# BSVogler/k8s-runpod-kubelet

Hardware: AMD Instinct MI355X
Metric: gpu_pods_scheduled_per_sec (higher is better)
Workload: dtype n/a; 1 GPU; podworker HIP init+kernel per pod (gfx950); model=gpu-pod-lifecycle, global_batch=1, seq_len=0, parallelism=1 kubelet x 1 GPUs, 8 sync workers, lifecycle=create->bind->launch->Ready->delete->finalized, burst_size=0, pods_total=10

## Files before the change

### k8s_runpod_kubelet_amd/ops/build.py

```python

from __future__ import annotations

import os
import shlex
import subprocess
import sys
import sysconfig
from pathlib import Path

OPS_DIR = Path(__file__).resolve().parent
CSRC = OPS_DIR / "csrc"
PODWORKER_DIR = OPS_DIR / "podworker"
GPUCHECK_DIR = OPS_DIR / "gpucheck"

GFX_ARCH = os.environ.get("PYTORCH_ROCM_ARCH", "gfx950")
HIPCC = os.environ.get("HIPCC", "/opt/rocm/bin/hipcc")
CXX = os.environ.get("CXX", "g++")


def _run(cmd: list[str]) -> None:
    print("+", " ".join(shlex.quote(c) for c in cmd), flush=True)
    subprocess.run(cmd, check=True)


def ext_suffix() -> str:
    return sysconfig.get_config_var("EXT_SUFFIX") or ".so"


def native_ext_path() -> Path:
    return OPS_DIR / f"_native{ext_suffix()}"


def podworker_path() -> Path:
    return PODWORKER_DIR / "podworker"


def gpucheck_path() -> Path:
    return GPUCHECK_DIR / "gpucheck"


def _content_stamp(sources: list[Path], cmd: list[str]) -> str:
    import hashlib

    h = hashlib.sha256()
    for s in sources:
        h.update(s.name.encode())
        h.update(s.read_bytes())
    h.update("\0".join(cmd).encode())
    return h.hexdigest()


def _is_fresh(target: Path, stamp_file: Path, stamp: str) -> bool:
    if not target.exists():
        return False
    try:
        return stamp_file.read_text().strip() == stamp
    except OSError:
        return False


def build_native(force: bool = False) -> Path:
    import pybind11

    out = native_ext_path()
    sources = [CSRC / "module.cpp", CSRC / "probe.cpp", CSRC / "launcher.cpp"]
    headers = [CSRC / "probe.h", CSRC / "launcher.h"]
    cmd = [
        CXX, "-O2", "-g", "-std=c++17", "-shared", "-fPIC",
        "-fvisibility=hidden",
        f"-I{pybind11.get_include()}",
        f"-I{sysconfig.get_paths()['include']}",
        *[str(s) for s in sources],
        "-o", str(out),
    ]
    stamp_file = OPS_DIR / ".native.buildstamp"
    stamp = _content_stamp(sources + headers, cmd)
    if not force and _is_fresh(out, stamp_file, stamp):
        return out
    _run(cmd)
    stamp_file.write_text(stamp + "\n")
    return out


def build_podworker(force: bool = False) -> Path:
    out = podworker_path()
    src = PODWORKER_DIR / "podworker.hip"
    cmd = [
        HIPCC, f"--offload-arch={GFX_ARCH}", "-O2", "-std=c++17",
        str(src), "-o", str(out),
    ]
    stamp_file = PODWORKER_DIR / ".podworker.buildstamp"
    stamp = _content_stamp([src], cmd)
    if not force and _is_fresh(out, stamp_file, stamp):
        return out
    _run(cmd)
    stamp_file.write_text(stamp + "\n")
    return out


def build_gpucheck(force: bool = False) -> Path:
    out = gpucheck_path()
    src = GPUCHECK_DIR / "gpucheck.hip"
    header = GPUCHECK_DIR / "gpucheck_pattern.h"
    cmd = [
        HIPCC, f"--offload-arch={GFX_ARCH}", "-O2", "-std=c++17",
        str(src), "-o", str(out),
    ]
    stamp_file = GPUCHECK_DIR / ".gpucheck.buildstamp"
    stamp = _content_stamp([src, header], cmd)
    if not force and _is_fresh(out, stamp_file, stamp):
        return out
    _run(cmd)
    stamp_file.write_text(stamp + "\n")
    return out


def build_all(force: bool = False) -> None:
    build_native(force=force)
    build_podworker(force=force)
    build_gpucheck(force=force)


if __name__ == "__main__":
    build_all(force="--force" in sys.argv)
```

### k8s_runpod_kubelet_amd/ops/podworker/podworker.hip

```cpp

#include <hip/hip_runtime.h>

#include <arpa/inet.h>
#include <netinet/in.h>
#include <signal.h>
#include <stdio.h>
#include <stdlib.h>
#include <string.h>
#include <sys/socket.h>
#include <time.h>
#include <unistd.h>

#include <string>
#include <vector>

#define HIP_CHECK(expr)                                                     \
  do {                                                                      \
    hipError_t err_ = (expr);                                               \
    if (err_ != hipSuccess) {                                               \
      fprintf(stderr, "podworker: %s failed: %s\n", #expr,                  \
              hipGetErrorString(err_));                                     \
      return 11;                                                            \
    }                                                                       \
  } while (0)

__global__ void touch_kernel(unsigned int* out, int n) {
  int i = blockIdx.x * blockDim.x + threadIdx.x;
  if (i < n) out[i] = static_cast<unsigned int>(i) * 2u + 1u;
}

static volatile sig_atomic_t g_terminate = 0;
static void on_term(int) { g_terminate = 1; }

static int touch_gpus(int expect_gpus) {
  int count = 0;
  HIP_CHECK(hipGetDeviceCount(&count));
  if (expect_gpus >= 0 && count != expect_gpus) {
    fprintf(stderr, "podworker: visible GPU count %d != expected %d\n", count,
            expect_gpus);
    return 12;
  }
  const int n = 1 << 20;
  for (int dev = 0; dev < count; ++dev) {
    HIP_CHECK(hipSetDevice(dev));
    unsigned int* d = nullptr;
    HIP_CHECK(hipMalloc(&d, n * sizeof(unsigned int)));
    dim3 block(256);
    dim3 grid((n + 255) / 256);
    hipLaunchKernelGGL(touch_kernel, grid, block, 0, 0, d, n);
    HIP_CHECK(hipGetLastError());
    const int head = 1 << 16;
    std::vector<unsigned int> host(head + 1);
    HIP_CHECK(hipMemcpy(host.data(), d, head * sizeof(unsigned int),
                        hipMemcpyDeviceToHost));
    HIP_CHECK(hipMemcpy(host.data() + head, d + (n - 1),
                        sizeof(unsigned int), hipMemcpyDeviceToHost));
    HIP_CHECK(hipFree(d));
    for (int i = 0; i < head; i += 4099) {
      if (host[i] != static_cast<unsigned int>(i) * 2u + 1u) {
        fprintf(stderr, "podworker: kernel verify failed at %d on dev %d\n", i,
                dev);
        return 13;
      }
    }
    if (host[head] != static_cast<unsigned int>(n - 1) * 2u + 1u) {
      fprintf(stderr, "podworker: kernel verify failed at tail on dev %d\n",
              dev);
      return 13;
    }
    hipDeviceProp_t prop;
    HIP_CHECK(hipGetDeviceProperties(&prop, dev));
    printf("podworker: dev %d %s gcnArch=%s vram=%zuMB ok\n", dev, prop.name,
           prop.gcnArchName, prop.totalGlobalMem >> 20);
  }
  return 0;
}

static int listen_on(int port) {
  int fd = socket(AF_INET, SOCK_STREAM | SOCK_CLOEXEC, 0);
  if (fd < 0) return -1;
  int one = 1;
  setsockopt(fd, SOL_SOCKET, SO_REUSEADDR, &one, sizeof(one));
  sockaddr_in addr{};
  addr.sin_family = AF_INET;
  addr.sin_addr.s_addr = htonl(INADDR_ANY);
  addr.sin_port = htons(static_cast<uint16_t>(port));
  if (bind(fd, reinterpret_cast<sockaddr*>(&addr), sizeof(addr)) != 0 ||
      listen(fd, 8) != 0) {
    close(fd);
    return -1;
  }
  return fd;
}

int main(int argc, char** argv) {
  int expect_gpus = -1;
  double run_for = -1.0;
  bool hold = false;
  int exit_code = 0;
  double startup_delay = 0.0;
  std::vector<int> ports;

  for (int i = 1; i < argc; ++i) {
    std::string a = argv[i];
    auto next = [&]() -> const char* { return (i + 1 < argc) ? argv[++i] : ""; };
    if (a == "--expect-gpus") expect_gpus = atoi(next());
    else if (a == "--run-for") run_for = atof(next());
    else if (a == "--hold") hold = true;
    else if (a == "--exit-code") exit_code = atoi(next());
    else if (a == "--startup-delay") startup_delay = atof(next());
    else if (a == "--listen-port") ports.push_back(atoi(next()));
    else if (a == "--fail") {
      fprintf(stderr, "podworker: simulated failure\n");
      return 1;
    } else {
      fprintf(stderr, "podworker: unknown arg %s\n", a.c_str());
      return 2;
    }
  }

  struct sigaction sa{};
  sa.sa_handler = on_term;
  sigaction(SIGTERM, &sa, nullptr);
  sigaction(SIGINT, &sa, nullptr);

  if (startup_delay > 0) usleep(static_cast<useconds_t>(startup_delay * 1e6));

  if (expect_gpus >= 0) {
    int rc = touch_gpus(expect_gpus);
    if (rc != 0) return rc;
  }

  std::vector<int> listen_fds;
  for (int p : ports) {
    int fd = listen_on(p);
    if (fd < 0) {
      fprintf(stderr, "podworker: listen on %d failed\n", p);
      return 3;
    }
    listen_fds.push_back(fd);
  }

  const char* ready_env = getenv("AMDVK_READY_FD");
  if (ready_env) {
    int fd = atoi(ready_env);
    const char msg[] = "READY\n";
    ssize_t w = write(fd, msg, sizeof(msg) - 1);
    (void)w;
    close(fd);
  }
  printf("podworker: ready (gpus=%d ports=%zu)\n", expect_gpus, ports.size());
  fflush(stdout);

  if (hold && run_for < 0) {
    while (!g_terminate) pause();
  } else if (run_for > 0) {
    double remaining = run_for;
    while (remaining > 0 && !g_terminate) {
      double chunk = remaining > 0.1 ? 0.1 : remaining;
      usleep(static_cast<useconds_t>(chunk * 1e6));
      remaining -= chunk;
    }
  }
  for (int fd : listen_fds) close(fd);
  printf("podworker: exiting code=%d\n", exit_code);
  return exit_code;
}
```

Measured before the change: 3.084 pods/s.

## Replace HIP runtime in podworker with direct HSA dispatch of embedded code object

The podworker no longer links the HIP runtime. It initializes HSA directly, loads a prebuilt code object embedded in the binary, and dispatches the touch kernel and a new gather kernel through AQL packets on one queue. Verification reads only the sampled elements from fine-grained host memory instead of copying them back with memcpy. The process exits via _exit to skip runtime teardown. The intent is to cut HIP runtime initialization and shutdown from each pod's startup and exit, at the cost of a more complex build (code-object extraction, metadata parsing) and hand-written queue and packet handling.

After: 3.676 pods/s (median of 6 runs). +19.2%, better.

```diff
diff --git a/k8s_runpod_kubelet_amd/ops/build.py b/k8s_runpod_kubelet_amd/ops/build.py
--- a/k8s_runpod_kubelet_amd/ops/build.py
+++ b/k8s_runpod_kubelet_amd/ops/build.py
@@ -82,18 +82,83 @@
     return out
 
 
+def _kernarg_offsets(notes: str) -> dict[str, list[int]]:
+    import re
+
+    kernels: dict[str, list[int]] = {}
+    body = notes.split("amdhsa.kernels:", 1)[1].split("\namdhsa.", 1)[0]
+    for block in re.split(r"^  - ", body, flags=re.M)[1:]:
+        name = re.search(r"^    \.name:\s+(\S+)", block, flags=re.M)
+        if not name:
+            raise RuntimeError("kernel metadata entry without a .name")
+        args = re.search(r"^    \.args:\n((?:      .*\n)*)", block, flags=re.M)
+        offsets = []
+        for arg in re.split(r"^      - ", args.group(1) if args else "",
+                            flags=re.M)[1:]:
+            if re.search(r"\.value_kind:\s+hidden_", arg):
+                continue
+            offsets.append(int(re.search(r"\.offset:\s+(\d+)", arg).group(1)))
+        kernels[name.group(1)] = offsets
+    return kernels
+
+
+def _write_kernels_inc(code_object: Path, notes: str, inc: Path) -> None:
+    offsets = _kernarg_offsets(notes)
+    expected = {"touch_kernel": 2, "gather_kernel": 4}
+    for name, nargs in expected.items():
+        if len(offsets.get(name, [])) != nargs:
+            raise RuntimeError(
+                f"{code_object.name}: expected {nargs} explicit arguments for "
+                f"{name}, metadata gives {offsets.get(name)}")
+    data = code_object.read_bytes()
+    lines = ["// generated by ops/build.py from podworker_kernels.hip",
+             "alignas(4096) static const unsigned char kPwCodeObject[] = {"]
+    for i in range(0, len(data), 16):
+        lines.append("  " + ",".join(str(b) for b in data[i:i + 16]) + ",")
+    lines.append("};")
+    for var, name in (("kTouchArgOffsets", "touch_kernel"),
+                      ("kGatherArgOffsets", "gather_kernel")):
+        lines.append(f"static const size_t {var}[] = "
+                     f"{{{', '.join(map(str, offsets[name]))}}};")
+    inc.write_text("\n".join(lines) + "\n")
+
+
 def build_podworker(force: bool = False) -> Path:
     out = podworker_path()
-    src = PODWORKER_DIR / "podworker.hip"
-    cmd = [
+    host_src = PODWORKER_DIR / "podworker.hip"
+    dev_src = PODWORKER_DIR / "podworker_kernels.hip"
+    code_object = PODWORKER_DIR / "podworker_kernels.co"
+    inc = PODWORKER_DIR / "podworker_kernels.inc"
+    staged = PODWORKER_DIR / "podworker.new"
+    readelf = subprocess.run(
+        [HIPCC, "-print-prog-name=llvm-readelf"], check=True,
+        capture_output=True, text=True).stdout.strip()
+    rocm = Path(os.environ.get("ROCM_PATH") or Path(readelf).resolve().parents[3])
+    rocm_lib = (rocm / "lib").resolve()
+    dev_cmd = [
         HIPCC, f"--offload-arch={GFX_ARCH}", "-O2", "-std=c++17",
-        str(src), "-o", str(out),
+        "--cuda-device-only", "--no-gpu-bundle-output",
+        str(dev_src), "-o", str(code_object),
+    ]
+    notes_cmd = [readelf, "--notes", str(code_object)]
+    host_cmd = [
+        CXX, "-O2", "-std=c++17", "-x", "c++", str(host_src), "-x", "none",
+        f"-I{rocm / 'include'}", f"-L{rocm_lib}", "-lhsa-runtime64",
+        f"-Wl,--enable-new-dtags,-rpath,{rocm_lib}",
+        "-o", str(staged),
     ]
     stamp_file = PODWORKER_DIR / ".podworker.buildstamp"
-    stamp = _content_stamp([src], cmd)
+    stamp = _content_stamp([host_src, dev_src],
+                           dev_cmd + notes_cmd + host_cmd)
     if not force and _is_fresh(out, stamp_file, stamp):
         return out
-    _run(cmd)
+    _run(dev_cmd)
+    print("+", " ".join(shlex.quote(c) for c in notes_cmd), flush=True)
+    notes = subprocess.run(notes_cmd, check=True, capture_output=True,
+                           text=True).stdout
+    _write_kernels_inc(code_object, notes, inc)
+    _run(host_cmd)
+    os.replace(staged, out)
     stamp_file.write_text(stamp + "\n")
     return out
 
diff --git a/k8s_runpod_kubelet_amd/ops/podworker/podworker.hip b/k8s_runpod_kubelet_amd/ops/podworker/podworker.hip
--- a/k8s_runpod_kubelet_amd/ops/podworker/podworker.hip
+++ b/k8s_runpod_kubelet_amd/ops/podworker/podworker.hip
@@ -1,9 +1,11 @@
 
-#include <hip/hip_runtime.h>
+#include <hsa/hsa.h>
+#include <hsa/hsa_ext_amd.h>
 
 #include <arpa/inet.h>
 #include <netinet/in.h>
 #include <signal.h>
+#include <stdint.h>
 #include <stdio.h>
 #include <stdlib.h>
 #include <string.h>
@@ -14,64 +16,367 @@
 #include <string>
 #include <vector>
 
-#define HIP_CHECK(expr)                                                     \
+#include "podworker_kernels.inc"
+
+[[noreturn]] static void finish(int code) {
+  fflush(stdout);
+  fflush(stderr);
+  _exit(code);
+}
+
+static const char* status_text(hsa_status_t st) {
+  const char* s = nullptr;
+  if (hsa_status_string(st, &s) == HSA_STATUS_SUCCESS && s) return s;
+  static char buf[32];
+  snprintf(buf, sizeof(buf), "HSA status 0x%x", static_cast<unsigned>(st));
+  return buf;
+}
+
+#define HSA_CHECK(expr)                                                     \
   do {                                                                      \
-    hipError_t err_ = (expr);                                               \
-    if (err_ != hipSuccess) {                                               \
+    hsa_status_t st_ = (expr);                                              \
+    if (st_ != HSA_STATUS_SUCCESS && st_ != HSA_STATUS_INFO_BREAK) {        \
       fprintf(stderr, "podworker: %s failed: %s\n", #expr,                  \
-              hipGetErrorString(err_));                                     \
-      return 11;                                                            \
+              status_text(st_));                                            \
+      finish(11);                                                           \
     }                                                                       \
   } while (0)
 
-__global__ void touch_kernel(unsigned int* out, int n) {
-  int i = blockIdx.x * blockDim.x + threadIdx.x;
-  if (i < n) out[i] = static_cast<unsigned int>(i) * 2u + 1u;
-}
-
 static volatile sig_atomic_t g_terminate = 0;
 static void on_term(int) { g_terminate = 1; }
 
-static int touch_gpus(int expect_gpus) {
-  int count = 0;
-  HIP_CHECK(hipGetDeviceCount(&count));
+static double now_ms() {
+  timespec ts;
+  clock_gettime(CLOCK_MONOTONIC, &ts);
+  return ts.tv_sec * 1e3 + ts.tv_nsec * 1e-6;
+}
+
+struct Timing {
+  double runtime_init = 0, queue = 0, load = 0, alloc = 0, dispatch_verify = 0;
+};
+
+static volatile int g_queue_error = 0;
+static volatile hsa_status_t g_queue_status = HSA_STATUS_SUCCESS;
+static void on_queue_error(hsa_status_t st, hsa_queue_t*, void*) {
+  fprintf(stderr, "podworker: queue error: %s\n", status_text(st));
+  g_queue_status = st;
+  g_queue_error = 1;
+}
+
+struct Agents {
+  std::vector<hsa_agent_t> gpus;
+  std::vector<hsa_agent_t> cpus;
+};
+
+static hsa_status_t collect_agent(hsa_agent_t agent, void* data) {
+  hsa_device_type_t type;
+  hsa_status_t st = hsa_agent_get_info(agent, HSA_AGENT_INFO_DEVICE, &type);
+  if (st != HSA_STATUS_SUCCESS) return st;
+  auto* a = static_cast<Agents*>(data);
+  if (type == HSA_DEVICE_TYPE_GPU) a->gpus.push_back(agent);
+  else if (type == HSA_DEVICE_TYPE_CPU) a->cpus.push_back(agent);
+  return HSA_STATUS_SUCCESS;
+}
+
+struct PoolQuery {
+  bool want_kernarg, want_fine, want_coarse;
+  bool found;
+  hsa_amd_memory_pool_t pool;
+};
+
+static hsa_status_t match_pool(hsa_amd_memory_pool_t pool, void* data) {
+  auto* q = static_cast<PoolQuery*>(data);
+  hsa_amd_segment_t seg;
+  hsa_status_t st = hsa_amd_memory_pool_get_info(
+      pool, HSA_AMD_MEMORY_POOL_INFO_SEGMENT, &seg);
+  if (st != HSA_STATUS_SUCCESS) return st;
+  if (seg != HSA_AMD_SEGMENT_GLOBAL) return HSA_STATUS_SUCCESS;
+  bool can_alloc = false;
+  st = hsa_amd_memory_pool_get_info(
+      pool, HSA_AMD_MEMORY_POOL_INFO_RUNTIME_ALLOC_ALLOWED, &can_alloc);
+  if (st != HSA_STATUS_SUCCESS) return st;
+  if (!can_alloc) return HSA_STATUS_SUCCESS;
+  uint32_t flags = 0;
+  st = hsa_amd_memory_pool_get_info(
+      pool, HSA_AMD_MEMORY_POOL_INFO_GLOBAL_FLAGS, &flags);
+  if (st != HSA_STATUS_SUCCESS) return st;
+  if (q->want_kernarg && !(flags & HSA_AMD_MEMORY_POOL_GLOBAL_FLAG_KERNARG_INIT))
+    return HSA_STATUS_SUCCESS;
+  if (q->want_fine && !(flags & HSA_AMD_MEMORY_POOL_GLOBAL_FLAG_FINE_GRAINED))
+    return HSA_STATUS_SUCCESS;
+  if (q->want_coarse &&
+      !(flags & HSA_AMD_MEMORY_POOL_GLOBAL_FLAG_COARSE_GRAINED))
+    return HSA_STATUS_SUCCESS;
+  q->pool = pool;
+  q->found = true;
+  return HSA_STATUS_INFO_BREAK;
+}
+
+static bool find_pool(const std::vector<hsa_agent_t>& agents, bool kernarg,
+                      bool fine, bool coarse, hsa_amd_memory_pool_t* out) {
+  for (hsa_agent_t a : agents) {
+    PoolQuery q{kernarg, fine, coarse, false, {}};
+    HSA_CHECK(hsa_amd_agent_iterate_memory_pools(a, match_pool, &q));
+    if (q.found) {
+      *out = q.pool;
+      return true;
+    }
+  }
+  return false;
+}
+
+static hsa_status_t first_isa(hsa_isa_t isa, void* data) {
+  *static_cast<hsa_isa_t*>(data) = isa;
+  return HSA_STATUS_INFO_BREAK;
+}
+
+struct Kernel {
+  uint64_t object = 0;
+  uint32_t kernarg_size = 0, group_size = 0, private_size = 0;
+};
+
+static Kernel lookup_kernel(hsa_executable_t exec, hsa_agent_t agent,
+                            const char* name) {
+  hsa_executable_symbol_t sym;
+  HSA_CHECK(hsa_executable_get_symbol_by_name(exec, name, &agent, &sym));
+  Kernel k;
+  HSA_CHECK(hsa_executable_symbol_get_info(
+      sym, HSA_EXECUTABLE_SYMBOL_INFO_KERNEL_OBJECT, &k.object));
+  HSA_CHECK(hsa_executable_symbol_get_info(
+      sym, HSA_EXECUTABLE_SYMBOL_INFO_KERNEL_KERNARG_SEGMENT_SIZE,
+      &k.kernarg_size));
+  HSA_CHECK(hsa_executable_symbol_get_info(
+      sym, HSA_EXECUTABLE_SYMBOL_INFO_KERNEL_GROUP_SEGMENT_SIZE,
+      &k.group_size));
+  HSA_CHECK(hsa_executable_symbol_get_info(
+      sym, HSA_EXECUTABLE_SYMBOL_INFO_KERNEL_PRIVATE_SEGMENT_SIZE,
+      &k.private_size));
+  return k;
+}
+
+template <typename T>
+static void put_arg(char* kernarg, const Kernel& k, size_t offset, T value) {
+  if (offset + sizeof(T) > k.kernarg_size) {
+    fprintf(stderr, "podworker: kernarg offset %zu past segment size %u\n",
+            offset, k.kernarg_size);
+    finish(11);
+  }
+  memcpy(kernarg + offset, &value, sizeof(T));
+}
+
+static const uint32_t kBlock = 256;
+static const uint32_t kQueuePackets = 64;
+static const unsigned int kPoison = 0xDEADBEEFu;
+
+static void fill_dispatch(hsa_kernel_dispatch_packet_t* p, const Kernel& k,
+                          uint32_t items, void* kernarg,
+                          hsa_signal_t completion) {
+  p->workgroup_size_x = kBlock;
+  p->workgroup_size_y = 1;
+  p->workgroup_size_z = 1;
+  p->reserved0 = 0;
+  p->grid_size_x = (items + kBlock - 1) / kBlock * kBlock;
+  p->grid_size_y = 1;
+  p->grid_size_z = 1;
+  p->private_segment_size = k.private_size;
+  p->group_segment_size = k.group_size;
+  p->kernel_object = k.object;
+  p->kernarg_address = kernarg;
+  p->reserved2 = 0;
+  p->completion_signal = completion;
+}
+
+static void publish(hsa_kernel_dispatch_packet_t* p, bool barrier) {
+  uint16_t header =
+      (HSA_PACKET_TYPE_KERNEL_DISPATCH << HSA_PACKET_HEADER_TYPE) |
+      ((barrier ? 1 : 0) << HSA_PACKET_HEADER_BARRIER) |
+      (HSA_FENCE_SCOPE_SYSTEM << HSA_PACKET_HEADER_SCACQUIRE_FENCE_SCOPE) |
+      (HSA_FENCE_SCOPE_SYSTEM << HSA_PACKET_HEADER_SCRELEASE_FENCE_SCOPE);
+  uint16_t setup = 1 << HSA_KERNEL_DISPATCH_PACKET_SETUP_DIMENSIONS;
+  __atomic_store_n(reinterpret_cast<uint32_t*>(p),
+                   header | (static_cast<uint32_t>(setup) << 16),
+                   __ATOMIC_RELEASE);
+}
+
+static int touch_gpus(int expect_gpus, int n, bool verify_all, Timing* tm) {
+  double t0 = now_ms();
+  HSA_CHECK(hsa_init());
+  Agents agents;
+  HSA_CHECK(hsa_iterate_agents(collect_agent, &agents));
+  int count = static_cast<int>(agents.gpus.size());
   if (expect_gpus >= 0 && count != expect_gpus) {
     fprintf(stderr, "podworker: visible GPU count %d != expected %d\n", count,
             expect_gpus);
     return 12;
   }
-  const int n = 1 << 20;
+  uint64_t ticks_per_s = 0;
+  HSA_CHECK(hsa_system_get_info(HSA_SYSTEM_INFO_TIMESTAMP_FREQUENCY,
+                                &ticks_per_s));
+  hsa_amd_memory_pool_t kernarg_pool{}, host_pool{};
+  if (count > 0) {
+    if (!find_pool(agents.cpus, true, false, false, &kernarg_pool)) {
+      fprintf(stderr, "podworker: kernarg pool lookup failed: none found\n");
+      return 11;
+    }
+    if (!find_pool(agents.cpus, false, true, false, &host_pool)) {
+      fprintf(stderr,
+              "podworker: fine-grained system pool lookup failed: none found\n");
+      return 11;
+    }
+  }
+  tm->runtime_init += now_ms() - t0;
+
+  std::vector<int> sample;
+  if (verify_all) {
+    sample.resize(n);
+    for (int i = 0; i < n; ++i) sample[i] = i;
+  } else {
+    const int head = n < (1 << 16) ? n : (1 << 16);
+    for (int i = 0; i < head; i += 4099) sample.push_back(i);
+    sample.push_back(n - 1);
+  }
+  const int m = static_cast<int>(sample.size());
+
   for (int dev = 0; dev < count; ++dev) {
-    HIP_CHECK(hipSetDevice(dev));
-    unsigned int* d = nullptr;
-    HIP_CHECK(hipMalloc(&d, n * sizeof(unsigned int)));
-    dim3 block(256);
-    dim3 grid((n + 255) / 256);
-    hipLaunchKernelGGL(touch_kernel, grid, block, 0, 0, d, n);
-    HIP_CHECK(hipGetLastError());
-    const int head = 1 << 16;
-    std::vector<unsigned int> host(head + 1);
-    HIP_CHECK(hipMemcpy(host.data(), d, head * sizeof(unsigned int),
-                        hipMemcpyDeviceToHost));
-    HIP_CHECK(hipMemcpy(host.data() + head, d + (n - 1),
-                        sizeof(unsigned int), hipMemcpyDeviceToHost));
-    HIP_CHECK(hipFree(d));
-    for (int i = 0; i < head; i += 4099) {
-      if (host[i] != static_cast<unsigned int>(i) * 2u + 1u) {
-        fprintf(stderr, "podworker: kernel verify failed at %d on dev %d\n", i,
-                dev);
+    hsa_agent_t gpu = agents.gpus[dev];
+
+    t0 = now_ms();
+    hsa_amd_memory_pool_t vram_pool{};
+    if (!find_pool({gpu}, false, false, true, &vram_pool)) {
+      fprintf(stderr,
+              "podworker: device memory pool lookup failed: none on dev %d\n",
+              dev);
+      return 11;
+    }
+    tm->runtime_init += now_ms() - t0;
+
+    t0 = now_ms();
+    hsa_queue_t* queue = nullptr;
+    HSA_CHECK(hsa_queue_create(gpu, kQueuePackets, HSA_QUEUE_TYPE_SINGLE,
+                               on_queue_error, nullptr, UINT32_MAX, UINT32_MAX,
+                               &queue));
+    tm->queue += now_ms() - t0;
+
+    t0 = now_ms();
+    hsa_code_object_reader_t reader;
+    HSA_CHECK(hsa_code_object_reader_create_from_memory(
+        kPwCodeObject, sizeof(kPwCodeObject), &reader));
+    hsa_executable_t exec;
+    HSA_CHECK(hsa_executable_create_alt(
+        HSA_PROFILE_FULL, HSA_DEFAULT_FLOAT_ROUNDING_MODE_DEFAULT, nullptr,
+        &exec));
+    HSA_CHECK(hsa_executable_load_agent_code_object(exec, gpu, reader, nullptr,
+                                                    nullptr));
+    HSA_CHECK(hsa_executable_freeze(exec, nullptr));
+    Kernel touch = lookup_kernel(exec, gpu, "touch_kernel.kd");
+    Kernel gather = lookup_kernel(exec, gpu, "gather_kernel.kd");
+    tm->load += now_ms() - t0;
+
+    t0 = now_ms();
+    unsigned int* out = nullptr;
+    int* idx = nullptr;
+    unsigned int* dst = nullptr;
+    char* kernarg = nullptr;
+    HSA_CHECK(hsa_amd_memory_pool_allocate(
+        vram_pool, static_cast<size_t>(n) * sizeof(unsigned int), 0,
+        reinterpret_cast<void**>(&out)));
+    HSA_CHECK(hsa_amd_memory_pool_allocate(
+        host_pool, static_cast<size_t>(m) * sizeof(int), 0,
+        reinterpret_cast<void**>(&idx)));
+    HSA_CHECK(hsa_amd_memory_pool_allocate(
+        host_pool, static_cast<size_t>(m) * sizeof(unsigned int), 0,
+        reinterpret_cast<void**>(&dst)));
+    const size_t gather_at = (touch.kernarg_size + 63u) & ~size_t(63);
+    const size_t kernarg_bytes = gather_at + gather.kernarg_size;
+    HSA_CHECK(hsa_amd_memory_pool_allocate(
+        kernarg_pool, kernarg_bytes, 0, reinterpret_cast<void**>(&kernarg)));
+    HSA_CHECK(hsa_amd_agents_allow_access(1, &gpu, nullptr, idx));
+    HSA_CHECK(hsa_amd_agents_allow_access(1, &gpu, nullptr, dst));
+    HSA_CHECK(hsa_amd_agents_allow_access(1, &gpu, nullptr, kernarg));
+    hsa_signal_t done;
+    HSA_CHECK(hsa_signal_create(1, 0, nullptr, &done));
+    tm->alloc += now_ms() - t0;
+
+    t0 = now_ms();
+    memcpy(idx, sample.data(), static_cast<size_t>(m) * sizeof(int));
+    for (int j = 0; j < m; ++j) dst[j] = kPoison;
+    memset(kernarg, 0, kernarg_bytes);
+    put_arg(kernarg, touch, kTouchArgOffsets[0], out);
+    put_arg(kernarg, touch, kTouchArgOffsets[1], n);
+    char* gather_args = kernarg + gather_at;
+    put_arg(gather_args, gather, kGatherArgOffsets[0],
+            static_cast<const unsigned int*>(out));
+    put_arg(gather_args, gather, kGatherArgOffsets[1],
+            static_cast<const int*>(idx));
+    put_arg(gather_args, gather, kGatherArgOffsets[2], dst);
+    put_arg(gather_args, gather, kGatherArgOffsets[3], m);
+
+    const uint64_t at = hsa_queue_add_write_index_relaxed(queue, 2);
+    auto* ring = static_cast<hsa_kernel_dispatch_packet_t*>(queue->base_address);
+    const uint32_t mask = queue->size - 1;
+    hsa_kernel_dispatch_packet_t* p0 = &ring[at & mask];
+    hsa_kernel_dispatch_packet_t* p1 = &ring[(at + 1) & mask];
+    fill_dispatch(p0, touch, static_cast<uint32_t>(n), kernarg,
+                  hsa_signal_t{0});
+    fill_dispatch(p1, gather, static_cast<uint32_t>(m), gather_args, done);
+    publish(p0, false);
+    publish(p1, true);
+    hsa_signal_store_screlease(queue->doorbell_signal,
+                               static_cast<hsa_signal_value_t>(at + 1));
+
+    const uint64_t slice = ticks_per_s / 10;
+    bool completed = false;
+    for (int s = 0; s < 100 && !g_queue_error; ++s) {
+      if (hsa_signal_wait_scacquire(done, HSA_SIGNAL_CONDITION_LT, 1, slice,
+                                    HSA_WAIT_STATE_BLOCKED) < 1) {
+        completed = true;
+        break;
+      }
+    }
+    if (g_queue_error) {
+      fprintf(stderr, "podworker: kernel dispatch failed: %s\n",
+              status_text(g_queue_status));
+      return 11;
+    }
+    if (!completed) {
+      fprintf(stderr,
+              "podworker: completion signal wait failed: timed out after 10 s\n");
+      return 11;
+    }
+
+    for (int j = 0; j < m; ++j) {
+      const int i = sample[j];
+      if (dst[j] != static_cast<unsigned int>(i) * 2u + 1u) {
+        if (!verify_all && j == m - 1)
+          fprintf(stderr, "podworker: kernel verify failed at tail on dev %d\n",
+                  dev);
+        else
+          fprintf(stderr, "podworker: kernel verify failed at %d on dev %d\n",
+                  i, dev);
         return 13;
       }
     }
-    if (host[head] != static_cast<unsigned int>(n - 1) * 2u + 1u) {
-      fprintf(stderr, "podworker: kernel verify failed at tail on dev %d\n",
-              dev);
-      return 13;
-    }
-    hipDeviceProp_t prop;
-    HIP_CHECK(hipGetDeviceProperties(&prop, dev));
-    printf("podworker: dev %d %s gcnArch=%s vram=%zuMB ok\n", dev, prop.name,
-           prop.gcnArchName, prop.totalGlobalMem >> 20);
+    tm->dispatch_verify += now_ms() - t0;
+
+    char product[64] = {0};
+    HSA_CHECK(hsa_agent_get_info(
+        gpu, static_cast<hsa_agent_info_t>(HSA_AMD_AGENT_INFO_PRODUCT_NAME),
+        product));
+    hsa_isa_t isa{};
+    HSA_CHECK(hsa_agent_iterate_isas(gpu, first_isa, &isa));
+    uint32_t isa_len = 0;
+    HSA_CHECK(hsa_isa_get_info_alt(isa, HSA_ISA_INFO_NAME_LENGTH, &isa_len));
+    std::string isa_name(isa_len + 1, '\0');
+    HSA_CHECK(hsa_isa_get_info_alt(isa, HSA_ISA_INFO_NAME, &isa_name[0]));
+    isa_name.resize(strlen(isa_name.c_str()));
+    const char prefix[] = "amdgcn-amd-amdhsa--";
+    if (isa_name.compare(0, sizeof(prefix) - 1, prefix) == 0)
+      isa_name.erase(0, sizeof(prefix) - 1);
+    size_t vram_bytes = 0;
+    HSA_CHECK(hsa_amd_memory_pool_get_info(
+        vram_pool, HSA_AMD_MEMORY_POOL_INFO_SIZE, &vram_bytes));
+    printf("podworker: dev %d %s gcnArch=%s vram=%zuMB ok\n", dev, product,
+           isa_name.c_str(), vram_bytes >> 20);
   }
   return 0;
 }
@@ -94,12 +399,15 @@
 }
 
 int main(int argc, char** argv) {
+  const double t_main = now_ms();
   int expect_gpus = -1;
   double run_for = -1.0;
   bool hold = false;
   int exit_code = 0;
   double startup_delay = 0.0;
   std::vector<int> ports;
+  long long touch_elems = 1 << 20;
+  bool verify_all = false;
 
   for (int i = 1; i < argc; ++i) {
     std::string a = argv[i];
@@ -110,13 +418,24 @@
     else if (a == "--exit-code") exit_code = atoi(next());
     else if (a == "--startup-delay") startup_delay = atof(next());
     else if (a == "--listen-port") ports.push_back(atoi(next()));
+    else if (a == "--touch-elems") touch_elems = atoll(next());
+    else if (a == "--verify-all") verify_all = true;
     else if (a == "--fail") {
       fprintf(stderr, "podworker: simulated failure\n");
-      return 1;
+      finish(1);
     } else {
       fprintf(stderr, "podworker: unknown arg %s\n", a.c_str());
-      return 2;
-    }
+      finish(2);
+    }
+  }
+  if (touch_elems < 1 || touch_elems > (1ll << 28)) {
+    fprintf(stderr, "podworker: --touch-elems must be in 1..%lld\n", 1ll << 28);
+    finish(2);
+  }
+  if (verify_all && touch_elems > (1 << 20)) {
+    fprintf(stderr, "podworker: --verify-all takes at most %d elements\n",
+            1 << 20);
+    finish(2);
   }
 
   struct sigaction sa{};
@@ -126,9 +445,11 @@
 
   if (startup_delay > 0) usleep(static_cast<useconds_t>(startup_delay * 1e6));
 
+  Timing tm;
   if (expect_gpus >= 0) {
-    int rc = touch_gpus(expect_gpus);
-    if (rc != 0) return rc;
+    int rc = touch_gpus(expect_gpus, static_cast<int>(touch_elems), verify_all,
+                        &tm);
+    if (rc != 0) finish(rc);
   }
 
   std::vector<int> listen_fds;
@@ -136,9 +457,17 @@
     int fd = listen_on(p);
     if (fd < 0) {
       fprintf(stderr, "podworker: listen on %d failed\n", p);
-      return 3;
+      finish(3);
     }
     listen_fds.push_back(fd);
+  }
+
+  const char* timing_env = getenv("AMDVK_PODWORKER_TIMING");
+  if (timing_env && strcmp(timing_env, "1") == 0) {
+    printf("podworker: timing runtime_init_ms=%.3f queue_ms=%.3f load_ms=%.3f "
+           "alloc_ms=%.3f dispatch_verify_ms=%.3f to_ready_ms=%.3f\n",
+           tm.runtime_init, tm.queue, tm.load, tm.alloc, tm.dispatch_verify,
+           now_ms() - t_main);
   }
 
   const char* ready_env = getenv("AMDVK_READY_FD");
@@ -164,5 +493,5 @@
   }
   for (int fd : listen_fds) close(fd);
   printf("podworker: exiting code=%d\n", exit_code);
-  return exit_code;
-}
+  finish(exit_code);
+}
diff --git a/k8s_runpod_kubelet_amd/ops/podworker/podworker_kernels.hip b/k8s_runpod_kubelet_amd/ops/podworker/podworker_kernels.hip
--- /dev/null
+++ b/k8s_runpod_kubelet_amd/ops/podworker/podworker_kernels.hip
@@ -0,0 +1,22 @@
+
+#include <hip/hip_runtime.h>
+
+#define PW_BLOCK 256
+
+static __device__ __forceinline__ int pw_global_index() {
+  return static_cast<int>(__builtin_amdgcn_workgroup_id_x()) * PW_BLOCK +
+         static_cast<int>(__builtin_amdgcn_workitem_id_x());
+}
+
+extern "C" __global__ void __launch_bounds__(PW_BLOCK)
+touch_kernel(unsigned int* out, int n) {
+  int i = pw_global_index();
+  if (i < n) out[i] = static_cast<unsigned int>(i) * 2u + 1u;
+}
+
+extern "C" __global__ void __launch_bounds__(PW_BLOCK)
+gather_kernel(const unsigned int* src, const int* idx, unsigned int* dst,
+              int m) {
+  int j = pw_global_index();
+  if (j < m) dst[j] = src[idx[j]];
+}
```
